# google-research/sparf

Hardware: AMD Instinct MI355X
Metric: training rays/sec (64c+128f samples, 8x256 MLP) (higher is better)
Workload: dtype bf16x3; 1 GPU; BASELINE configs[1]: DTU-shaped scene, fixed GT poses, photometric loss; 4 views 300x400, 4096 rays x (64 coarse + 128 fine) per GPU and step, fwd+bwd+clip+Adam, both 8x256 MLPs; samples=64+128, precision_mode=bf16x3, launch=eager, optimizer=clip_grad_norm(0.1) + Adam, sparf_amd.optim.FusedAdam

## Files before the change

sparf_amd/build.py:

```python
import os
import subprocess
import sys

HERE = os.path.dirname(os.path.abspath(__file__))
CSRC = os.path.join(HERE, "csrc")
OUT = os.path.join(HERE, "libsparf_hip.so")
FUSED_UNITS = ["mlp_fwd_fp32_train.hip", "mlp_fwd_fp32_infer.hip", "rays_fwd_fp32.hip", "rays_bwd_fp32.hip", "mlp_fwd_x3_train.hip", "rays_fwd_x3.hip", "mlp_fwd_x3_train_q8.hip", "mlp_fwd_x3_infer.hip", "mlp_bwd.hip", "mlp_bwd_fp32.hip", "mlp_bwd_x3.hip", "mlp_bwd_x3w4.hip", "mlp_bwd_q8.hip", "rays_bwd_x3.hip", "rays_bwd_x3w4.hip", "rays_bwd.hip", "rays_fwd_bf16.hip",
               "mlp_fwd_bf16_train.hip", "mlp_fwd_bf16_train_q8.hip", "mlp_fwd_bf16_infer.hip"]
RAYS_UNITS = ["rays_fwd_fp32.hip", "rays_bwd_fp32.hip", "rays_fwd_x3.hip", "rays_bwd_x3.hip", "rays_bwd_x3w4.hip", "rays_bwd.hip", "rays_fwd_bf16.hip"]
MLP_DISPATCH = "mlp_launch.hip"
SOURCES = FUSED_UNITS + ["wgrad.hip", "api.hip", MLP_DISPATCH, "ray_ops.hip", "pose.hip", "pose_eval.hip", "reproj.hip", "dcons.hip", "photo.hip", "matches.hip", "colmap.hip", "depth_err.hip", "pick.hip", "metrics.hip", "pack.hip", "optim.hip", "calib.hip", "tables.cpp"]
HEADERS = ["layout.h", "streams.h", "mlp_dev.h", "mlp_fwd_impl.h", "mlp_bwd_impl.h", "kernels.h", "pass_plan.h", "ordered.h", "reproj.h", "dcons.h", "photo.h", "matches.h", "colmap.h", "depth_err.h", "pick.h", "metrics.h", "pose_eval.h", "rigid.h", os.path.join("..", "..", "include", "sparf_hip.h")]
FLAGS = ["--offload-arch=gfx950", "-O3", "-std=c++17", "-fPIC", "-ffp-contract=on", "-fconstexpr-steps=200000000"]


def source_hash():
    import hashlib
    h = hashlib.sha1()
    for f in sorted(SOURCES) + sorted(HEADERS):
        h.update(open(os.path.join(CSRC, f), "rb").read())
    return h.hexdigest()[:16]


def _deps(path, seen=None):
    import re
    seen = set() if seen is None else seen
    if path in seen or not os.path.exists(path):
        return seen
    seen.add(path)
    for inc in re.findall(r'^\s*#\s*include\s+"([^"]+)"', open(path, errors="replace").read(), flags=re.M):
        _deps(os.path.normpath(os.path.join(os.path.dirname(path), inc)), seen)
    return seen


def _newer(target, deps):
    if not os.path.exists(target):
        return True
    t = os.path.getmtime(target)
    return any(os.path.getmtime(d) > t for d in deps)


def build(force=False, verbose=True, out=None, extra_flags=(), tag="", only=None):
    hipcc = os.environ.get("HIPCC", "/opt/rocm/bin/hipcc")
    bdir = os.path.join(CSRC, "build" + tag)
    out = out or OUT
    os.makedirs(bdir, exist_ok=True)
    hdrs = [os.path.join(CSRC, h) for h in HEADERS]
    procs, objs = [], []
    for src in SOURCES:
        sp = os.path.join(CSRC, src)
        if only is not None and src not in only:
            objs.append(os.path.join(CSRC, "build", os.path.splitext(src)[0] + ".o"))
            continue
        obj = os.path.join(bdir, os.path.splitext(src)[0] + ".o")
        objs.append(obj)
        if force or _newer(obj, sorted(_deps(sp))):
            cmd = [hipcc] + FLAGS + list(extra_flags) + (["-x", "hip"] if src.endswith(".cpp") else []) + ["-c", sp, "-o", obj]
            if verbose:
                print("[sparf_amd.build]", " ".join(cmd), flush=True)
            procs.append((src, subprocess.Popen(cmd, stdout=subprocess.PIPE, stderr=subprocess.STDOUT, text=True)))
    failed = []
    for src, p in procs:
        log, _ = p.communicate()
        if p.returncode != 0:
            failed.append((src, log))
# ... 14 lines not shown
```

sparf_amd/csrc/optim.hip:

```cpp
#include "kernels.h"
#include "layout.h"

namespace sparf {

enum { OPT_BLOCK = 256, OPT_PARTS = 256 };

__global__ void __launch_bounds__(OPT_BLOCK) grad_sqnorm_kernel(const float* __restrict__ g, int n, float* __restrict__ parts, int* __restrict__ step_dev) {
    if (step_dev && blockIdx.x == 0 && threadIdx.x == 0) *step_dev += 1;
    if (!parts) return;
    float s = 0.f;
    for (int i = blockIdx.x * OPT_BLOCK + threadIdx.x; i < n; i += OPT_PARTS * OPT_BLOCK) s += g[i] * g[i];
    __shared__ float red[OPT_BLOCK];
    red[threadIdx.x] = s;
    __syncthreads();
    for (int k = OPT_BLOCK / 2; k > 0; k >>= 1) {
        if ((int)threadIdx.x < k) red[threadIdx.x] += red[threadIdx.x + k];
        __syncthreads();
    }
    if (threadIdx.x == 0) parts[blockIdx.x] = red[0];
}

struct OptPtrs { float* p[2 * N_LAYERS]; };

struct AdamArgs {
    OptPtrs p;
    const float* grad;
    float* exp_avg;
    float* exp_avg_sq;
    const float* parts;
    float* norm_out;
    float lr, beta1, beta2, eps, bias1, bias2_sqrt, max_norm;
    const int* step_dev;
};

__global__ void __launch_bounds__(OPT_BLOCK) adam_kernel(AdamArgs a) {
    __shared__ int off[2 * N_LAYERS + 1];
    __shared__ float* ptr[2 * N_LAYERS];
    __shared__ float clip, sh_bias1, sh_bias2_sqrt;
    if (threadIdx.x == 1) {
        float b1 = a.bias1, b2s = a.bias2_sqrt;
        if (a.step_dev) {
            const double st = (double)*a.step_dev;
            b1 = (float)(1.0 - pow((double)a.beta1, st));
            b2s = (float)sqrt(1.0 - pow((double)a.beta2, st));
        }
        sh_bias1 = b1; sh_bias2_sqrt = b2s;
    }
    if (threadIdx.x < 2 * N_LAYERS + 1) {
        const int k = threadIdx.x;
        off[k] = k == 2 * N_LAYERS ? (int)N_PARAMS : (int)((k & 1) ? param_b_off(k >> 1) : param_w_off(k >> 1));
    }
#pragma unroll
    for (int k = 0; k < 2 * N_LAYERS; ++k)
        if ((int)threadIdx.x == k + 32) ptr[k] = a.p.p[k];
    if (threadIdx.x == 0) {
        float c = 1.0f;
        if (a.parts) {
            float s = 0.f;
            for (int i = 0; i < OPT_PARTS; ++i) s += a.parts[i];
            const float norm = sqrtf(s);
            c = fminf(a.max_norm / (norm + 1e-6f), 1.0f);
            if (a.norm_out && blockIdx.x == 0) *a.norm_out = norm;
        }
        clip = c;
    }
    __syncthreads();
    const int i = blockIdx.x * OPT_BLOCK + threadIdx.x;
    if (i >= N_PARAMS) return;
    int k = 0;
#pragma unroll
    for (int step = 16; step > 0; step >>= 1)
        if (k + step <= 2 * N_LAYERS && off[k + step] <= i) k += step;
    float* w = ptr[k] + (i - off[k]);
    const float g = a.grad[i] * clip;
    const float m = a.exp_avg[i] + (1.0f - a.beta1) * (g - a.exp_avg[i]);
    const float v = a.beta2 * a.exp_avg_sq[i] + (1.0f - a.beta2) * g * g;
    a.exp_avg[i] = m;
    a.exp_avg_sq[i] = v;
    const float denom = sqrtf(v) / sh_bias2_sqrt + a.eps;
    *w = *w - (a.lr / sh_bias1) * (m / denom);
}

int launch_adam(const float* const* params, const float* grad, float* exp_avg, float* exp_avg_sq, float* workspace, float* norm_out,
                float lr, float beta1, float beta2, float eps, int step, int* step_dev, float max_norm, hipStream_t s) {
    AdamArgs a;
    for (int i = 0; i < 2 * N_LAYERS; ++i) a.p.p[i] = const_cast<float*>(params[i]);
    a.grad = grad; a.exp_avg = exp_avg; a.exp_avg_sq = exp_avg_sq;
    a.parts = nullptr; a.norm_out = norm_out;
    a.lr = lr; a.beta1 = beta1; a.beta2 = beta2; a.eps = eps; a.max_norm = max_norm;
    a.step_dev = step_dev;
    a.bias1 = (float)(1.0 - pow((double)beta1, (double)(step > 0 ? step : 1)));
    a.bias2_sqrt = (float)sqrt(1.0 - pow((double)beta2, (double)(step > 0 ? step : 1)));
    if (max_norm > 0.0f || step_dev) {
        hipLaunchKernelGGL(grad_sqnorm_kernel, dim3(max_norm > 0.0f ? OPT_PARTS : 1), dim3(OPT_BLOCK), 0, s, grad, (int)N_PARAMS,
                           max_norm > 0.0f ? workspace : (float*)nullptr, step_dev);
        if (max_norm > 0.0f) a.parts = workspace;
    }
    hipLaunchKernelGGL(adam_kernel, dim3((N_PARAMS + OPT_BLOCK - 1) / OPT_BLOCK), dim3(OPT_BLOCK), 0, s, a);
    return hipGetLastError() == hipSuccess ? 0 : 2;
}


enum { PHOTO_BLOCK = 1024, PHOTO_PARTS = 256, PHOTO_SINGLE_MAX = 65536 };

__global__ void __launch_bounds__(PHOTO_BLOCK) photometric_loss_kernel(const float* __restrict__ pred, const float* __restrict__ pred_fine,
                                                                       const float* __restrict__ target, int64_t n, int kind, float delta,
                                                                       float* __restrict__ out, float* __restrict__ d_pred,
                                                                       float* __restrict__ d_pred_fine, int final_scale) {
    const float inv = kind == 0 ? (float)(1.0 / ((double)n + 1e-6)) : (float)(2.0 / (double)n);
    float s = 0.f;
    for (int64_t i = (int64_t)blockIdx.x * PHOTO_BLOCK + threadIdx.x; i < n; i += (int64_t)gridDim.x * PHOTO_BLOCK) {
        const float t = target[i];
#pragma unroll
        for (int f = 0; f < 2; ++f) {
            const float* p = f ? pred_fine : pred;
            float* d = f ? d_pred_fine : d_pred;
            if (!p) continue;
            const float e = p[i] - t;
            float l, g;
            if (kind == 0) { l = e * e; g = 2.0f * e; }
            else if (fabsf(e) <= delta) { l = 0.5f * e * e; g = e; }
            else { l = delta * (fabsf(e) - 0.5f * delta); g = e > 0.f ? delta : -delta; }
            s += l;
            if (d) d[i] = g * inv;
        }
    }
    __shared__ float red[PHOTO_BLOCK];
    red[threadIdx.x] = s;
    __syncthreads();
    for (int k = PHOTO_BLOCK / 2; k > 0; k >>= 1) {
        if ((int)threadIdx.x < k) red[threadIdx.x] += red[threadIdx.x + k];
        __syncthreads();
    }
    if (threadIdx.x == 0) out[blockIdx.x] = final_scale ? red[0] * inv : red[0];
}

__global__ void __launch_bounds__(PHOTO_PARTS) photometric_final_kernel(const float* __restrict__ parts, int nparts, int64_t n, int kind,
                                                                        float* __restrict__ loss) {
    __shared__ float red[PHOTO_PARTS];
    red[threadIdx.x] = (int)threadIdx.x < nparts ? parts[threadIdx.x] : 0.f;
    __syncthreads();
    for (int k = PHOTO_PARTS / 2; k > 0; k >>= 1) {
        if ((int)threadIdx.x < k) red[threadIdx.x] += red[threadIdx.x + k];
        __syncthreads();
    }
    if (threadIdx.x == 0) *loss = red[0] * (kind == 0 ? (float)(1.0 / ((double)n + 1e-6)) : (float)(2.0 / (double)n));
}

int photometric_workspace_floats() { return PHOTO_PARTS; }

int launch_photometric_loss(const float* pred, const float* pred_fine, const float* target, int64_t n, int kind, float delta,
// ... 17 lines not shown
```

sparf_amd/csrc/ray_ops.hip:

```cpp
#include "kernels.h"
#include "mlp_dev.h"

namespace sparf {

static SP_DEV double wave_incl_scan(double v, int lane) {
#pragma unroll
    for (int d = 1; d < 64; d <<= 1) {
        double o = __shfl_up(v, d);
        if (lane >= d) v += o;
    }
    return v;
}
static SP_DEV double wave_rev_incl_scan(double v, int lane) {
#pragma unroll
    for (int d = 1; d < 64; d <<= 1) {
        double o = __shfl_down(v, d);
        if (lane + d < 64) v += o;
    }
    return v;
}
static SP_DEV double wave_sum(double v) {
#pragma unroll
    for (int d = 32; d >= 1; d >>= 1) v += __shfl_xor(v, d);
    return v;
}
static SP_DEV float wave_sumf(float v) {
#pragma unroll
    for (int d = 32; d >= 1; d >>= 1) v += __shfl_xor(v, d);
    return v;
}
static SP_DEV float softplus_f(float x) { return x > 20.0f ? x : log1pf(expf(x)); }
static SP_DEV float sigmoid_f(float x) { return 1.0f / (1.0f + expf(-x)); }

template <int PREC>
__global__ void ray_setup_kernel(const float* __restrict__ dir, int nrays, const float* __restrict__ c2f_view,
                                 typename Policy<PREC>::stage_t* __restrict__ venc, float* __restrict__ raylen) {
    typedef typename Policy<PREC>::stage_t act_t;
    constexpr int CH = Policy<PREC>::CH;
    int ray = blockIdx.x * blockDim.x + threadIdx.x;
    if (ray >= nrays) return;
    float x = dir[ray * 3], y = dir[ray * 3 + 1], z = dir[ray * 3 + 2];
    float len = sqrtf(__fadd_rn(__fadd_rn(__fmul_rn(x, x), __fmul_rn(y, y)), __fmul_rn(z, z)));
    raylen[ray] = len;
    float inv = fmaxf(len, 1e-12f);
    float d[3] = {x / inv, y / inv, z / inv};
    float feat[V_DIM];
    feat[0] = d[0]; feat[1] = d[1]; feat[2] = d[2];
    for (int c = 0; c < 3; ++c)
        for (int k = 0; k < LVIEW; ++k) {
            float s, co;
            sincosf(__fmul_rn(d[c], pe_freq(k)), &s, &co);
            feat[3 + c * 8 + k] = __fmul_rn(s, c2f_view[k]);
            feat[3 + c * 8 + 4 + k] = __fmul_rn(co, c2f_view[k]);
        }
    act_t* o = venc + (int64_t)ray * 32;
    for (int h = 0; h < 2; ++h)
        for (int q = 0; q < 16; ++q) {
            int f = view_feat(q, h);
            o[pos_of(q, h, CH)] = (act_t)(f < 0 ? 0.0f : feat[f]);
        }
}

__global__ void sample_coarse_kernel(const float* __restrict__ jitter, float u_const, const float* __restrict__ dmax_ray,
                                     const float* __restrict__ range_dev, float dmin, float scale, int inverse, int64_t rows,
                                     int nsamp, float* __restrict__ t) {
    int64_t i = (int64_t)blockIdx.x * blockDim.x + threadIdx.x;
    if (i >= rows) return;
    if (range_dev) {
        dmin = range_dev[0];
        if (!dmax_ray) scale = __fsub_rn(range_dev[1], dmin);
    }
    int s = (int)(i % nsamp);
    float u = jitter ? jitter[i] : u_const;
    float sc = dmax_ray ? __fsub_rn(dmax_ray[i / nsamp], dmin) : scale;
    float v = __fadd_rn(__fmul_rn(__fdiv_rn(__fadd_rn(u, (float)s), (float)nsamp), sc), dmin);
    if (inverse) v = __fdiv_rn(1.0f, __fadd_rn(v, 1e-8f));
    t[i] = v;
}

struct SegPick {
    int ray0; float noise_scale; const float *g_rgb, *g_depth, *g_opacity, *g_weights;
    const float *g_depth_var, *g_rgb_var, *g_all_cum, *g_density, *g_rgb_samples;
};
static SP_DEV SegPick pick_segment(const SegTable& st, int ray, const SegPick& pass_level) {
    SegPick p = pass_level;
    if (st.n > 0) {
#pragma unroll
        for (int s = 0; s < MAX_SEGMENTS; ++s)
            if (s < st.n && ray >= st.ray0[s])
                p = SegPick{st.ray0[s], st.noise_scale[s], st.g_rgb[s], st.g_depth[s], st.g_opacity[s], st.g_weights[s],
                            st.g_depth_var[s], st.g_rgb_var[s], st.g_all_cum[s], st.g_density[s], st.g_rgb_samples[s]};
    }
    return p;
}

__global__ void __launch_bounds__(64) composite_fwd_kernel(CompositeFwdArgs a) {
    const int ray = blockIdx.x, lane = threadIdx.x;
    const int N = a.nsamp;
    const int64_t base = (int64_t)ray * N;
    const float ell = a.raylen[ray];
    const float noise_scale = pick_segment(a.seg, ray, SegPick{0, a.noise_scale, nullptr, nullptr, nullptr, nullptr, nullptr, nullptr, nullptr, nullptr, nullptr}).noise_scale;
    double carry = 0.0;
    float s_w = 0.f, s_d = 0.f, s_r = 0.f, s_g = 0.f, s_b = 0.f;
    float T_nm2 = 1.0f;
    for (int j0 = 0; j0 < N; j0 += 64) {
        const int i = j0 + lane;
        const bool ok = i < N;
        float sd = 0.f, tt = 0.f, dens = 0.f;
        if (ok) {
            tt = a.t[base + i];
            float tn = i + 1 < N ? a.t[base + i + 1] : 0.f;
            float delta = i + 1 < N ? __fsub_rn(tn, tt) : 1e10f;
            float raw = a.sigma_raw[base + i];
            if (a.noise && noise_scale != 0.0f) raw = __fadd_rn(raw, __fmul_rn(a.noise[base + i], noise_scale));
            dens = a.direct ? raw : softplus_f(raw);
            sd = __fmul_rn(dens, __fmul_rn(delta, ell));
        }
        double incl = wave_incl_scan((double)sd, lane);
        double excl = carry + incl - (double)sd;
        carry += __shfl(incl, 63);
        if (ok) {
            float T = expf(-(float)excl);
            float alpha = 1.0f - expf(-sd);
            float w = T * alpha;
            a.weights[base + i] = w;
            if (a.density) a.density[base + i] = dens;
            if (i == N - 2) T_nm2 = T;
            const float* c = a.rgb_samples + (base + i) * 3;
            s_w += w; s_d += w * tt; s_r += w * c[0]; s_g += w * c[1]; s_b += w * c[2];
        }
    }
    const float opacity = wave_sumf(s_w), depth = wave_sumf(s_d);
    const float r = wave_sumf(s_r), g = wave_sumf(s_g), b = wave_sumf(s_b);
    float Tn = (N >= 2 && ((N - 2) % 64) == lane) ? T_nm2 : 0.f;
    Tn = wave_sumf(Tn);
    float v_d = 0.f, v_c = 0.f;
    for (int j0 = 0; j0 < N; j0 += 64) {
        const int i = j0 + lane;
        if (i < N) {
            float w = a.weights[base + i], tt = a.t[base + i];
            const float* c = a.rgb_samples + (base + i) * 3;
            float dd = tt - depth;
            v_d += w * dd * dd;
            v_c += w * ((c[0] - r) + (c[1] - g) + (c[2] - b));
        }
    }
    v_d = wave_sumf(v_d); v_c = wave_sumf(v_c);
    if (lane == 0) {
        float add = a.white_bg ? 1.0f - opacity : 0.0f;
        a.rgb[ray * 3 + 0] = r + add; a.rgb[ray * 3 + 1] = g + add; a.rgb[ray * 3 + 2] = b + add;
        a.depth[ray] = depth; a.opacity[ray] = opacity; a.depth_var[ray] = v_d; a.rgb_var[ray] = v_c;
        a.all_cumulated[ray] = Tn;
    }
}

__global__ void __launch_bounds__(64) composite_bwd_kernel(CompositeBwdArgs a) {
    const int ray = a.ray_base + blockIdx.x, lane = threadIdx.x;
    const int N = a.nsamp;
    const int64_t base = (int64_t)ray * N;
    const float ell = a.raylen[ray];
    const SegPick sg = pick_segment(a.seg, ray, SegPick{0, a.noise_scale, a.g_rgb, a.g_depth, a.g_opacity, a.g_weights,
                                                      a.g_depth_var, a.g_rgb_var, a.g_all_cum, a.g_density, a.g_rgb_samples});
    const int lray = ray - sg.ray0;
    const float noise_scale = sg.noise_scale;
    const float* gw = sg.g_weights ? sg.g_weights + (int64_t)lray * N : nullptr;
    const float* gdn = sg.g_density ? sg.g_density + (int64_t)lray * N : nullptr;
    const float* grs = sg.g_rgb_samples ? sg.g_rgb_samples + (int64_t)lray * N * 3 : nullptr;
    float gC[3] = {0.f, 0.f, 0.f}, gD = 0.f, gO = 0.f;
    if (sg.g_rgb) { gC[0] = sg.g_rgb[lray * 3]; gC[1] = sg.g_rgb[lray * 3 + 1]; gC[2] = sg.g_rgb[lray * 3 + 2]; }
    if (sg.g_depth) gD = sg.g_depth[lray];
    if (sg.g_opacity) gO = sg.g_opacity[lray];
    if (a.white_bg) gO -= gC[0] + gC[1] + gC[2];
    const float gV = sg.g_depth_var ? sg.g_depth_var[lray] : 0.f, gU = sg.g_rgb_var ? sg.g_rgb_var[lray] : 0.f;
    const float gA = sg.g_all_cum ? sg.g_all_cum[lray] : 0.f;
    float Dr = 0.f, Or = 0.f, SC = 0.f;
    if (sg.g_depth_var || sg.g_rgb_var) {
        for (int i = lane; i < N; i += 64) {
            const float w = a.weights[base + i];
            const float* c = a.rgb_samples + (base + i) * 3;
            Dr += w * a.t[base + i]; Or += w; SC += w * (c[0] + c[1] + c[2]);
        }
        Dr = wave_sumf(Dr); Or = wave_sumf(Or); SC = wave_sumf(SC);
    }
    double carry_sd = 0.0;
    float A_part = 0.f;
    for (int j0 = 0; j0 < N; j0 += 64) {
        const int i = j0 + lane;
        float sd = 0.f;
        if (i < N) {
            const float tt = a.t[base + i];
            const float delta = i + 1 < N ? __fsub_rn(a.t[base + i + 1], tt) : 1e10f;
            float raw = a.sigma_raw[base + i];
            if (a.noise && noise_scale != 0.0f) raw = __fadd_rn(raw, __fmul_rn(a.noise[base + i], noise_scale));
            sd = __fmul_rn(a.direct ? raw : softplus_f(raw), __fmul_rn(delta, ell));
        }
        double incl_sd = carry_sd + wave_incl_scan((double)sd, lane);
        carry_sd = __shfl(incl_sd, 63);
        if (i < N) {
            const float Tn = expf(-(float)incl_sd);
            a.d_sigma_raw[base + i] = Tn;
            if (i == N - 3) A_part = Tn;
        }
    }
    const float A = sg.g_all_cum ? (N >= 3 ? wave_sumf(A_part) : N == 2 ? 1.0f : 0.0f) : 0.0f;
    double carry = 0.0;
    float dlen = 0.f;
    for (int j0 = ((N - 1) / 64) * 64; j0 >= 0; j0 -= 64) {
        const int i = j0 + lane;
        const bool ok = i < N;
        float w = 0.f, q = 0.f, tt = 0.f, dens = 0.f, delta = 0.f, raw = 0.f, Tn1 = 0.f;
        const float* c = a.rgb_samples + (base + (ok ? i : 0)) * 3;
        if (ok) {
            tt = a.t[base + i];
            w = a.weights[base + i];
            q = gC[0] * c[0] + gC[1] * c[1] + gC[2] * c[2] + gD * tt + gO + (gw ? gw[i] : 0.f);
            if (sg.g_depth_var) q += gV * ((tt - Dr) * (tt - Dr) - 2.0f * tt * Dr * (1.0f - Or));
            if (sg.g_rgb_var) q += gU * ((c[0] + c[1] + c[2]) * (1.0f - Or) - SC);
            float tn = i + 1 < N ? a.t[base + i + 1] : 0.f;
            delta = i + 1 < N ? __fsub_rn(tn, tt) : 1e10f;
            raw = a.sigma_raw[base + i];
            if (a.noise && noise_scale != 0.0f) raw = __fadd_rn(raw, __fmul_rn(a.noise[base + i], noise_scale));
            dens = a.direct ? raw : softplus_f(raw);
            Tn1 = a.d_sigma_raw[base + i];
        }
        const double wq = (double)w * (double)q;
        const double rincl = wave_rev_incl_scan(wq, lane);
        const double rnext = __shfl_down(rincl, 1);
        const double suffix_d = carry + (lane < 63 ? rnext : 0.0);
        carry += __shfl(rincl, 0);
        if (ok) {
            float suffix = (float)suffix_d;
            float ds = Tn1 * q - suffix;
            if (i < N - 2) ds -= gA * A;
            float dist = delta * ell;
            float dsig = ds * dist + (gdn ? gdn[i] : 0.f);
            float draw = a.direct ? dsig : dsig * (raw > 20.0f ? 1.0f : sigmoid_f(raw));
            a.d_sigma_raw[base + i] = draw;
            dlen += ds * dens * delta;
            float* dz = a.d_z + (base + i) * 3;
            const float wu = w * gU * (1.0f - Or);
#pragma unroll
            for (int ch = 0; ch < 3; ++ch) {
                const float dc = w * gC[ch] + wu + (grs ? grs[i * 3 + ch] : 0.f);
                dz[ch] = a.direct ? dc : dc * c[ch] * (1.0f - c[ch]);
            }
        }
    }
    dlen = wave_sumf(dlen);
    if (lane == 0 && a.d_len) a.d_len[ray] = dlen;
}

static SP_DEV float linspace_at(float start, float end, int steps, int i) {
    float step = (end - start) / (float)(steps - 1);
    return i < steps / 2 ? __fadd_rn(start, __fmul_rn(step, (float)i)) : __fsub_rn(end, __fmul_rn(step, (float)(steps - i - 1)));
}

__global__ void __launch_bounds__(64) sample_fine_kernel(SampleFineArgs a) {
    extern __shared__ float sm[];
    const int ray = blockIdx.x, lane = threadIdx.x;
    const int Nc = a.n_coarse, Nf = a.n_fine, Nt = Nc + Nf;
    float* cdf = sm;
    float* srt = sm + (Nc + 1);
    int P = 1;
    while (P < Nt) P <<= 1;
    const float* w = a.weights + (int64_t)ray * Nc;
    const float dmin = a.range_dev ? a.range_dev[0] : a.dmin, dmax = a.range_dev ? a.range_dev[1] : a.dmax;
    double tot = 0.0;
    for (int i = lane; i < Nc; i += 64) tot += (double)w[i];
    const float denom = __fadd_rn((float)wave_sum(tot), 1e-6f);
    double carry = 0.0;
    if (lane == 0) cdf[0] = 0.f;
    for (int j0 = 0; j0 < Nc; j0 += 64) {
        const int i = j0 + lane;
        float pdf = i < Nc ? __fdiv_rn(w[i], denom) : 0.f;
        double incl = carry + wave_incl_scan((double)pdf, lane);
        carry = __shfl(incl, 63);
        if (i < Nc) cdf[i + 1] = (float)incl;
    }
    __syncthreads();
    const float* tc = a.t_coarse + (int64_t)ray * Nc;
    for (int i = lane; i < Nc; i += 64) srt[i] = tc[i];
    for (int j = lane; j < Nf; j += 64) {
        const float u = a.u_mid ? a.u_mid[j] : a.u_host[j];
        int lo = 0, hi = Nc + 1;
        while (lo < hi) {
            int mid = (lo + hi) >> 1;
            if (cdf[mid] <= u) lo = mid + 1; else hi = mid;
        }
        const int il = lo - 1 < 0 ? 0 : lo - 1, ih = lo > Nc ? Nc : lo;
        const float dl = linspace_at(dmin, dmax, Nc + 1, il), dh = linspace_at(dmin, dmax, Nc + 1, ih);
        const float cl = cdf[il], chh = cdf[ih];
        const float frac = __fdiv_rn(__fsub_rn(u, cl), __fadd_rn(__fsub_rn(chh, cl), 1e-8f));
        const float tf = __fadd_rn(dl, __fmul_rn(frac, __fsub_rn(dh, dl)));
        srt[Nc + j] = tf;
        if (a.t_fine) a.t_fine[(int64_t)ray * Nf + j] = tf;
    }
    for (int i = Nt + lane; i < P; i += 64) srt[i] = __builtin_inff();
    __syncthreads();
    for (int k = 2; k <= P; k <<= 1)
        for (int j = k >> 1; j > 0; j >>= 1) {
            for (int i = lane; i < P; i += 64) {
                int p = i ^ j;
                if (p > i) {
                    float x = srt[i], y = srt[p];
                    bool up = (i & k) == 0;
                    if ((x > y) == up) { srt[i] = y; srt[p] = x; }
                }
            }
            __syncthreads();
        }
    float* out = a.t_out + (int64_t)ray * Nt;
    for (int i = lane; i < Nt; i += 64) out[i] = srt[i];
}

__global__ void __launch_bounds__(64) ray_reduce_kernel(RayReduceArgs a) {
    const int ray = a.ray_base + blockIdx.x, lane = threadIdx.x;
    const int N = a.nsamp;
    const int64_t base = (int64_t)ray * N;
    float sc[3] = {0, 0, 0}, sr[3] = {0, 0, 0};
    for (int i = lane; i < N; i += 64) {
        const float* dp = a.dp + (base + i) * 3;
        float tt = a.t[base + i];
#pragma unroll
        for (int c = 0; c < 3; ++c) { sc[c] += dp[c]; sr[c] += tt * dp[c]; }
    }
#pragma unroll
    for (int c = 0; c < 3; ++c) { sc[c] = wave_sumf(sc[c]); sr[c] = wave_sumf(sr[c]); }
    float dvf = 0.f;
    if (a.dv) {
        const int hh = lane >> 5, col = lane & 31;
        float s0 = 0.f, s1 = 0.f, s2 = 0.f, s3 = 0.f;
        int i = hh;
        for (; i + 6 < N; i += 8) {
            s0 += a.dv[(base + i) * 32 + col];
            s1 += a.dv[(base + i + 2) * 32 + col];
            s2 += a.dv[(base + i + 4) * 32 + col];
            s3 += a.dv[(base + i + 6) * 32 + col];
        }
        for (; i < N; i += 2) s0 += a.dv[(base + i) * 32 + col];
        dvf = (s0 + s1) + (s2 + s3);
        dvf += __shfl_down(dvf, 32);
    }
    float x = a.dir[ray * 3], y = a.dir[ray * 3 + 1], z = a.dir[ray * 3 + 2];
    float len = a.raylen[ray];
    float inv = fmaxf(len, 1e-12f);
    float d[3] = {x / inv, y / inv, z / inv};
    float gd[3] = {0, 0, 0};
    if (a.dv) {
        float contrib = 0.f;
        int coord = -1;
        const int feat = lane < 32 ? view_feat(q_of_pos(lane, 4), h_of_pos(lane, 4)) : -1;
        if (feat >= 0 && feat < 3) { coord = feat; contrib = dvf; }
        else if (feat >= 3) {
            int f = feat - 3; coord = f / 8;
            int k = f % 4; bool is_cos = (f % 8) >= 4;
            float s, co;
            sincosf(__fmul_rn(d[coord], pe_freq(k)), &s, &co);
            float m = a.c2f_view[k] * pe_freq(k);
            contrib = dvf * m * (is_cos ? -s : co);
        }
#pragma unroll
        for (int c = 0; c < 3; ++c) gd[c] = wave_sumf(coord == c ? contrib : 0.f);
    }
    if (lane == 0) {
// ... 61 lines not shown
}

int launch_far_transplant(int main_prec, bool masks, const void* far_area, void* main_area, int64_t frows, int far_count, int nsamp, hipStream_t s) {
    if (frows <= 0) return 0;
    if (main_prec == PREC_FP32) return 1;
    const int64_t ntiles = (frows + 31) / 32;
    hipLaunchKernelGGL(far_transplant_kernel, dim3((unsigned)ntiles), dim3(256), 0, s, (const char*)far_area, (char*)main_area, frows, far_count, nsamp,
                       save_tile_bytes(masks ? (int)AREA_MASKS : main_prec), save_mask_tile_off(masks ? (int)AREA_MASKS : main_prec, 0), masks ? 1 : 0);
    return hipGetLastError() == hipSuccess ? 0 : 2;
}

__global__ void ray_len_kernel(const float* __restrict__ dir, int nrays, float* __restrict__ raylen) {
    int ray = blockIdx.x * blockDim.x + threadIdx.x;
    if (ray >= nrays) return;
    float x = dir[ray * 3], y = dir[ray * 3 + 1], z = dir[ray * 3 + 2];
    raylen[ray] = sqrtf(__fadd_rn(__fadd_rn(__fmul_rn(x, x), __fmul_rn(y, y)), __fmul_rn(z, z)));
}
__global__ void len_to_dir_kernel(const float* __restrict__ dir, const float* __restrict__ raylen, const float* __restrict__ d_len, int nrays,
                                  float* __restrict__ d_dir) {
    int ray = blockIdx.x * blockDim.x + threadIdx.x;
    if (ray >= nrays) return;
    const float inv = fmaxf(raylen[ray], 1e-12f), g = d_len[ray];
#pragma unroll
    for (int c = 0; c < 3; ++c) d_dir[ray * 3 + c] = g * dir[ray * 3 + c] / inv;
}
int launch_len_to_dir(const float* dir, const float* raylen, const float* d_len, int nrays, float* d_dir, hipStream_t s) {
    if (nrays <= 0) return 0;
    hipLaunchKernelGGL(len_to_dir_kernel, dim3((nrays + 255) / 256), dim3(256), 0, s, dir, raylen, d_len, nrays, d_dir);
    return hipGetLastError() == hipSuccess ? 0 : 2;
}

int launch_ray_setup(int prec, const float* dir, int nrays, const float* c2f_view, void* venc, float* raylen, hipStream_t s) {
    if (nrays <= 0) return 0;
    dim3 g((nrays + 255) / 256), b(256);
    if (prec < 0) {
        hipLaunchKernelGGL(ray_len_kernel, g, b, 0, s, dir, nrays, raylen);
        return hipGetLastError() == hipSuccess ? 0 : 2;
    }
    if (prec == PREC_BF16) hipLaunchKernelGGL(ray_setup_kernel<PREC_BF16>, g, b, 0, s, dir, nrays, c2f_view, (__bf16*)venc, raylen);
    else if (prec == PREC_FP32) hipLaunchKernelGGL(ray_setup_kernel<PREC_FP32>, g, b, 0, s, dir, nrays, c2f_view, (float*)venc, raylen);
    else if (prec == PREC_X3) hipLaunchKernelGGL(ray_setup_kernel<PREC_X3>, g, b, 0, s, dir, nrays, c2f_view, (float*)venc, raylen);
    else return 1;
    return hipGetLastError() == hipSuccess ? 0 : 2;
}
int launch_sample_coarse(const float* jitter, float u_const, const float* dmax_ray, const float* range_dev, float dmin, float scale,
                         int inverse, int64_t rows, int nsamp, float* t, hipStream_t s) {
    if (rows <= 0) return 0;
    hipLaunchKernelGGL(sample_coarse_kernel, dim3((unsigned)((rows + 255) / 256)), dim3(256), 0, s, jitter, u_const, dmax_ray, range_dev,
                       dmin, scale, inverse, rows, nsamp, t);
    return hipGetLastError() == hipSuccess ? 0 : 2;
}
int launch_composite_fwd(const CompositeFwdArgs& a, hipStream_t s) {
    if (a.nrays <= 0) return 0;
    hipLaunchKernelGGL(composite_fwd_kernel, dim3(a.nrays), dim3(64), 0, s, a);
    return hipGetLastError() == hipSuccess ? 0 : 2;
}
int launch_composite_bwd(const CompositeBwdArgs& a, hipStream_t s) {
    if (a.nrays <= 0) return 0;
    hipLaunchKernelGGL(composite_bwd_kernel, dim3(a.nrays), dim3(64), 0, s, a);
    return hipGetLastError() == hipSuccess ? 0 : 2;
}
int launch_sample_fine(const SampleFineArgs& a, hipStream_t s) {
    if (a.nrays <= 0) return 0;
    int P = 1;
    while (P < a.n_coarse + a.n_fine) P <<= 1;
    size_t smem = (size_t)(a.n_coarse + 1 + P) * sizeof(float);
    if (smem > 64 * 1024) return 3;
    hipLaunchKernelGGL(sample_fine_kernel, dim3(a.nrays), dim3(64), smem, s, a);
    return hipGetLastError() == hipSuccess ? 0 : 2;
}
int launch_ray_reduce(const RayReduceArgs& a, hipStream_t s) {
    if (a.nrays <= 0) return 0;
    hipLaunchKernelGGL(ray_reduce_kernel, dim3(a.nrays), dim3(64), 0, s, a);
    return hipGetLastError() == hipSuccess ? 0 : 2;
}


struct RayGeom { float ki[9], ri[9], ti[3]; };

static SP_DEV RayGeom ray_geom(const float* pose, const float* intr, int b) {
    RayGeom g;
    const float* K = intr + b * 9;
    const double a = K[0], bb = K[1], c = K[2], d = K[3], e = K[4], f = K[5], gg = K[6], h = K[7], i = K[8];
    const double A = e * i - f * h, B = -(d * i - f * gg), C = d * h - e * gg;
    const double det = a * A + bb * B + c * C, inv = 1.0 / det;
    g.ki[0] = (float)(A * inv); g.ki[1] = (float)(-(bb * i - c * h) * inv); g.ki[2] = (float)((bb * f - c * e) * inv);
    g.ki[3] = (float)(B * inv); g.ki[4] = (float)((a * i - c * gg) * inv);  g.ki[5] = (float)(-(a * f - c * d) * inv);
    g.ki[6] = (float)(C * inv); g.ki[7] = (float)(-(a * h - bb * gg) * inv); g.ki[8] = (float)((a * e - bb * d) * inv);
    const float* P = pose + b * 12;
#pragma unroll
    for (int r = 0; r < 3; ++r)
#pragma unroll
        for (int q = 0; q < 3; ++q) g.ri[r * 3 + q] = P[q * 4 + r];
#pragma unroll
    for (int r = 0; r < 3; ++r) g.ti[r] = -(g.ri[r * 3] * P[3] + g.ri[r * 3 + 1] * P[7] + g.ri[r * 3 + 2] * P[11]);
    return g;
}

static SP_DEV void ray_pixel(const RayGenArgs& a, int b, int r, float& x, float& y) {
    const int64_t src = (a.per_image ? (int64_t)b * a.nrays : 0) + r;
    if (a.pixels) {
        x = a.pixels[src * 2];
        y = a.pixels[src * 2 + 1];
    } else {
        const int64_t idx = a.ray_idx[src];
        x = (float)(idx % a.width) + 0.5f;
        y = (float)(idx / a.width) + 0.5f;
    }
}

__global__ void ray_gen_fwd_kernel(RayGenArgs a) {
    const int b = blockIdx.y;
// ... 72 lines not shown
```

Baseline: 626,400 rays/s.

## Vectorize Adam, register-resident multi-ray compositing, merge-based fine sample sort

Adam now handles four elements per thread with 16-byte vector loads and stores, and the first wave reads the gradient-norm partials in parallel instead of one thread summing them serially. Forward and backward compositing are templated on the number of 64-sample chunks, keep per-sample data in registers, and pack four rays per workgroup; sample counts above 256 fall back to the old loop kernel. Fine sampling replaces the full bitonic sort of coarse plus fine samples with a check that both runs are already sorted, followed by a binary-search merge-rank scatter, and keeps the bitonic sort as a fallback. These changes target launch granularity, repeated global reads and sort work, at the cost of more register pressure and extra code paths.

```diff
diff --git a/sparf_amd/build.py b/sparf_amd/build.py
--- a/sparf_amd/build.py
+++ b/sparf_amd/build.py
@@ -10,7 +10,7 @@
 RAYS_UNITS = ["rays_fwd_fp32.hip", "rays_bwd_fp32.hip", "rays_fwd_x3.hip", "rays_bwd_x3.hip", "rays_bwd_x3w4.hip", "rays_bwd.hip", "rays_fwd_bf16.hip"]
 MLP_DISPATCH = "mlp_launch.hip"
 SOURCES = FUSED_UNITS + ["wgrad.hip", "api.hip", MLP_DISPATCH, "ray_ops.hip", "pose.hip", "pose_eval.hip", "reproj.hip", "dcons.hip", "photo.hip", "matches.hip", "colmap.hip", "depth_err.hip", "pick.hip", "metrics.hip", "pack.hip", "optim.hip", "calib.hip", "tables.cpp"]
-HEADERS = ["layout.h", "streams.h", "mlp_dev.h", "mlp_fwd_impl.h", "mlp_bwd_impl.h", "kernels.h", "pass_plan.h", "ordered.h", "reproj.h", "dcons.h", "photo.h", "matches.h", "colmap.h", "depth_err.h", "pick.h", "metrics.h", "pose_eval.h", "rigid.h", os.path.join("..", "..", "include", "sparf_hip.h")]
+HEADERS = ["layout.h", "streams.h", "mlp_dev.h", "mlp_fwd_impl.h", "mlp_bwd_impl.h", "kernels.h", "pass_plan.h", "ordered.h", "merge_rank.h", "reproj.h", "dcons.h", "photo.h", "matches.h", "colmap.h", "depth_err.h", "pick.h", "metrics.h", "pose_eval.h", "rigid.h", os.path.join("..", "..", "include", "sparf_hip.h")]
 FLAGS = ["--offload-arch=gfx950", "-O3", "-std=c++17", "-fPIC", "-ffp-contract=on", "-fconstexpr-steps=200000000"]
 
 
diff --git a/sparf_amd/csrc/merge_rank.h b/sparf_amd/csrc/merge_rank.h
--- /dev/null
+++ b/sparf_amd/csrc/merge_rank.h
@@ -0,0 +1,18 @@
+#pragma once
+#include "layout.h"
+
+namespace sparf {
+
+SP_HD bool merge_run_ok(float v, bool last, float next) { return v == v && v != 0.0f && (last || v <= next); }
+
+SP_HD int merge_rank(const float* run, int n, float v, bool strict) {
+    int lo = 0, hi = n;
+    while (lo < hi) {
+        const int mid = (lo + hi) >> 1;
+        const float x = run[mid];
+        if (strict ? x < v : x <= v) lo = mid + 1; else hi = mid;
+    }
+    return lo;
+}
+
+}
diff --git a/sparf_amd/csrc/optim.hip b/sparf_amd/csrc/optim.hip
--- a/sparf_amd/csrc/optim.hip
+++ b/sparf_amd/csrc/optim.hip
@@ -3,7 +3,9 @@
 
 namespace sparf {
 
-enum { OPT_BLOCK = 256, OPT_PARTS = 256 };
+enum { OPT_BLOCK = 256, OPT_PARTS = 256, ADAM_VEC = 4 };
+static_assert(N_PARAMS % ADAM_VEC == 0, "adam_kernel reads whole vectors of the flat buffers");
+static_assert(OPT_PARTS % 64 == 0, "adam_kernel's first wave holds the partials, OPT_PARTS / 64 a lane");
 
 __global__ void __launch_bounds__(OPT_BLOCK) grad_sqnorm_kernel(const float* __restrict__ g, int n, float* __restrict__ parts, int* __restrict__ step_dev) {
     if (step_dev && blockIdx.x == 0 && threadIdx.x == 0) *step_dev += 1;
@@ -33,11 +35,54 @@
     const int* step_dev;
 };
 
+typedef float f32x4 __attribute__((ext_vector_type(4)));
+
+static __device__ __forceinline__ float adam_element(const AdamArgs& a, float clip, float bias1, float bias2_sqrt, float grad, float w, float& exp_avg, float& exp_avg_sq) {
+    const float g = grad * clip;
+    const float m = exp_avg + (1.0f - a.beta1) * (g - exp_avg);
+    const float v = a.beta2 * exp_avg_sq + (1.0f - a.beta2) * g * g;
+    exp_avg = m;
+    exp_avg_sq = v;
+    const float denom = sqrtf(v) / bias2_sqrt + a.eps;
+    return w - (a.lr / bias1) * (m / denom);
+}
+
+static __device__ __forceinline__ bool aligned16(const void* p) { return ((uintptr_t)p & 15) == 0; }
+
 __global__ void __launch_bounds__(OPT_BLOCK) adam_kernel(AdamArgs a) {
     __shared__ int off[2 * N_LAYERS + 1];
     __shared__ float* ptr[2 * N_LAYERS];
     __shared__ float clip, sh_bias1, sh_bias2_sqrt;
-    if (threadIdx.x == 1) {
+    const int tid = threadIdx.x;
+    const int i0 = (blockIdx.x * OPT_BLOCK + tid) * ADAM_VEC;
+    const bool live = i0 < N_PARAMS;
+    const bool flat16 = aligned16(a.grad) && aligned16(a.exp_avg) && aligned16(a.exp_avg_sq);
+    f32x4 g = {0.f, 0.f, 0.f, 0.f}, m = g, v = g;
+    if (live) {
+        if (flat16) {
+            g = *(const f32x4*)(a.grad + i0); m = *(const f32x4*)(a.exp_avg + i0); v = *(const f32x4*)(a.exp_avg_sq + i0);
+        } else {
+#pragma unroll
+            for (int e = 0; e < ADAM_VEC; ++e) { g[e] = a.grad[i0 + e]; m[e] = a.exp_avg[i0 + e]; v[e] = a.exp_avg_sq[i0 + e]; }
+        }
+    }
+    if (tid < 64) {
+        float c = 1.0f;
+        if (a.parts) {
+            float pv[OPT_PARTS / 64];
+#pragma unroll
+            for (int j = 0; j < OPT_PARTS / 64; ++j) pv[j] = a.parts[j * 64 + tid];
+            float s = 0.f;
+#pragma unroll
+            for (int j = 0; j < OPT_PARTS / 64; ++j)
+#pragma unroll
+                for (int l = 0; l < 64; ++l) s += __int_as_float(__builtin_amdgcn_readlane(__float_as_int(pv[j]), l));
+            const float norm = sqrtf(s);
+            c = fminf(a.max_norm / (norm + 1e-6f), 1.0f);
+            if (tid == 0 && a.norm_out && blockIdx.x == 0) *a.norm_out = norm;
+        }
+        if (tid == 0) clip = c;
+    } else if (tid == 64) {
         float b1 = a.bias1, b2s = a.bias2_sqrt;
         if (a.step_dev) {
             const double st = (double)*a.step_dev;
@@ -45,40 +90,55 @@
             b2s = (float)sqrt(1.0 - pow((double)a.beta2, st));
         }
         sh_bias1 = b1; sh_bias2_sqrt = b2s;
-    }
-    if (threadIdx.x < 2 * N_LAYERS + 1) {
-        const int k = threadIdx.x;
+    } else if (tid >= 128 && tid < 128 + 2 * N_LAYERS + 1) {
+        const int k = tid - 128;
         off[k] = k == 2 * N_LAYERS ? (int)N_PARAMS : (int)((k & 1) ? param_b_off(k >> 1) : param_w_off(k >> 1));
     }
 #pragma unroll
     for (int k = 0; k < 2 * N_LAYERS; ++k)
-        if ((int)threadIdx.x == k + 32) ptr[k] = a.p.p[k];
-    if (threadIdx.x == 0) {
-        float c = 1.0f;
-        if (a.parts) {
-            float s = 0.f;
-            for (int i = 0; i < OPT_PARTS; ++i) s += a.parts[i];
-            const float norm = sqrtf(s);
-            c = fminf(a.max_norm / (norm + 1e-6f), 1.0f);
-            if (a.norm_out && blockIdx.x == 0) *a.norm_out = norm;
-        }
-        clip = c;
-    }
-    __syncthreads();
-    const int i = blockIdx.x * OPT_BLOCK + threadIdx.x;
-    if (i >= N_PARAMS) return;
+        if (tid == k + 192) ptr[k] = a.p.p[k];
+    __syncthreads();
+    if (!live) return;
+    const float cl = clip, bias1 = sh_bias1, bias2_sqrt = sh_bias2_sqrt;
     int k = 0;
 #pragma unroll
     for (int step = 16; step > 0; step >>= 1)
-        if (k + step <= 2 * N_LAYERS && off[k + step] <= i) k += step;
-    float* w = ptr[k] + (i - off[k]);
-    const float g = a.grad[i] * clip;
-    const float m = a.exp_avg[i] + (1.0f - a.beta1) * (g - a.exp_avg[i]);
-    const float v = a.beta2 * a.exp_avg_sq[i] + (1.0f - a.beta2) * g * g;
-    a.exp_avg[i] = m;
-    a.exp_avg_sq[i] = v;
-    const float denom = sqrtf(v) / sh_bias2_sqrt + a.eps;
-    *w = *w - (a.lr / sh_bias1) * (m / denom);
+        if (k + step <= 2 * N_LAYERS && off[k + step] <= i0) k += step;
+    if (i0 + ADAM_VEC <= off[k + 1]) {
+        float* w = ptr[k] + (i0 - off[k]);
+        const bool w16 = aligned16(w);
+        f32x4 wv;
+        if (w16) wv = *(const f32x4*)w;
+        else {
+#pragma unroll
+            for (int e = 0; e < ADAM_VEC; ++e) wv[e] = w[e];
+        }
+#pragma unroll
+        for (int e = 0; e < ADAM_VEC; ++e) {
+            float me = m[e], ve = v[e];
+            wv[e] = adam_element(a, cl, bias1, bias2_sqrt, g[e], wv[e], me, ve);
+            m[e] = me; v[e] = ve;
+        }
+        if (w16) *(f32x4*)w = wv;
+        else {
+#pragma unroll
+            for (int e = 0; e < ADAM_VEC; ++e) w[e] = wv[e];
+        }
+    } else {
+#pragma unroll
+        for (int e = 0; e < ADAM_VEC; ++e) {
+            while (off[k + 1] <= i0 + e) ++k;
+            float* w = ptr[k] + (i0 + e - off[k]);
+            float me = m[e], ve = v[e];
+            *w = adam_element(a, cl, bias1, bias2_sqrt, g[e], *w, me, ve);
+            m[e] = me; v[e] = ve;
+        }
+    }
+    if (flat16) { *(f32x4*)(a.exp_avg + i0) = m; *(f32x4*)(a.exp_avg_sq + i0) = v; }
+    else {
+#pragma unroll
+        for (int e = 0; e < ADAM_VEC; ++e) { a.exp_avg[i0 + e] = m[e]; a.exp_avg_sq[i0 + e] = v[e]; }
+    }
 }
 
 int launch_adam(const float* const* params, const float* grad, float* exp_avg, float* exp_avg_sq, float* workspace, float* norm_out,
@@ -96,7 +156,7 @@
                            max_norm > 0.0f ? workspace : (float*)nullptr, step_dev);
         if (max_norm > 0.0f) a.parts = workspace;
     }
-    hipLaunchKernelGGL(adam_kernel, dim3((N_PARAMS + OPT_BLOCK - 1) / OPT_BLOCK), dim3(OPT_BLOCK), 0, s, a);
+    hipLaunchKernelGGL(adam_kernel, dim3((N_PARAMS + OPT_BLOCK * ADAM_VEC - 1) / (OPT_BLOCK * ADAM_VEC)), dim3(OPT_BLOCK), 0, s, a);
     return hipGetLastError() == hipSuccess ? 0 : 2;
 }
 
diff --git a/sparf_amd/csrc/ray_ops.hip b/sparf_amd/csrc/ray_ops.hip
--- a/sparf_amd/csrc/ray_ops.hip
+++ b/sparf_amd/csrc/ray_ops.hip
@@ -1,5 +1,6 @@
 #include "kernels.h"
 #include "mlp_dev.h"
+#include "merge_rank.h"
 
 namespace sparf {
 
@@ -94,7 +95,91 @@
     return p;
 }
 
-__global__ void __launch_bounds__(64) composite_fwd_kernel(CompositeFwdArgs a) {
+enum { COMPOSITE_REG_CHUNKS = 4, COMPOSITE_RAYS_PER_WG = 4 };
+
+template <int C>
+__global__ void __launch_bounds__(64 * COMPOSITE_RAYS_PER_WG) composite_fwd_kernel(CompositeFwdArgs a) {
+    const int lane = threadIdx.x & 63;
+    const int ray = blockIdx.x * COMPOSITE_RAYS_PER_WG + __builtin_amdgcn_readfirstlane(threadIdx.x >> 6);
+    if (ray >= a.nrays) return;
+    const int N = a.nsamp;
+    const int64_t base = (int64_t)ray * N;
+    const float ell = a.raylen[ray];
+    const float noise_scale = pick_segment(a.seg, ray, SegPick{0, a.noise_scale, nullptr, nullptr, nullptr, nullptr, nullptr, nullptr, nullptr, nullptr, nullptr}).noise_scale;
+    const bool noisy = a.noise && noise_scale != 0.0f;
+    float tt[C], tn[C], raw[C], nz[C], col[C][3];
+#pragma unroll
+    for (int k = 0; k < C; ++k) {
+        const int i = k * 64 + lane, ic = i < N ? i : N - 1;
+        tt[k] = a.t[base + ic];
+        tn[k] = a.t[base + (ic + 1 < N ? ic + 1 : ic)];
+        raw[k] = a.sigma_raw[base + ic];
+        const float* c = a.rgb_samples + (base + ic) * 3;
+        col[k][0] = c[0]; col[k][1] = c[1]; col[k][2] = c[2];
+    }
+#pragma unroll
+    for (int k = 0; k < C; ++k) {
+        const int i = k * 64 + lane;
+        nz[k] = noisy ? a.noise[base + (i < N ? i : N - 1)] : 0.f;
+    }
+    if (noisy)
+#pragma unroll
+        for (int k = 0; k < C; ++k) raw[k] = __fadd_rn(raw[k], __fmul_rn(nz[k], noise_scale));
+    double carry = 0.0;
+    float s_w = 0.f, s_d = 0.f, s_r = 0.f, s_g = 0.f, s_b = 0.f;
+    float T_nm2 = 1.0f;
+    float wv[C];
+#pragma unroll
+    for (int k = 0; k < C; ++k) {
+        const int i = k * 64 + lane;
+        const bool ok = i < N;
+        float sd = 0.f, dens = 0.f;
+        if (ok) {
+            float delta = i + 1 < N ? __fsub_rn(tn[k], tt[k]) : 1e10f;
+            dens = a.direct ? raw[k] : softplus_f(raw[k]);
+            sd = __fmul_rn(dens, __fmul_rn(delta, ell));
+        }
+        double incl = wave_incl_scan((double)sd, lane);
+        double excl = carry + incl - (double)sd;
+        carry += __shfl(incl, 63);
+        wv[k] = 0.f;
+        if (ok) {
+            float T = expf(-(float)excl);
+            float alpha = 1.0f - expf(-sd);
+            float w = T * alpha;
+            a.weights[base + i] = w;
+            if (a.density) a.density[base + i] = dens;
+            if (i == N - 2) T_nm2 = T;
+            const float* c = col[k];
+            s_w += w; s_d += w * tt[k]; s_r += w * c[0]; s_g += w * c[1]; s_b += w * c[2];
+            wv[k] = w;
+        }
+    }
+    const float opacity = wave_sumf(s_w), depth = wave_sumf(s_d);
+    const float r = wave_sumf(s_r), g = wave_sumf(s_g), b = wave_sumf(s_b);
+    float Tn = (N >= 2 && ((N - 2) % 64) == lane) ? T_nm2 : 0.f;
+    Tn = wave_sumf(Tn);
+    float v_d = 0.f, v_c = 0.f;
+#pragma unroll
+    for (int k = 0; k < C; ++k) {
+        if (k * 64 + lane < N) {
+            float w = wv[k];
+            const float* c = col[k];
+            float dd = tt[k] - depth;
+            v_d += w * dd * dd;
+            v_c += w * ((c[0] - r) + (c[1] - g) + (c[2] - b));
+        }
+    }
+    v_d = wave_sumf(v_d); v_c = wave_sumf(v_c);
+    if (lane == 0) {
+        float add = a.white_bg ? 1.0f - opacity : 0.0f;
+        a.rgb[ray * 3 + 0] = r + add; a.rgb[ray * 3 + 1] = g + add; a.rgb[ray * 3 + 2] = b + add;
+        a.depth[ray] = depth; a.opacity[ray] = opacity; a.depth_var[ray] = v_d; a.rgb_var[ray] = v_c;
+        a.all_cumulated[ray] = Tn;
+    }
+}
+
+__global__ void __launch_bounds__(64) composite_fwd_loop_kernel(CompositeFwdArgs a) {
     const int ray = blockIdx.x, lane = threadIdx.x;
     const int N = a.nsamp;
     const int64_t base = (int64_t)ray * N;
@@ -154,7 +239,128 @@
     }
 }
 
-__global__ void __launch_bounds__(64) composite_bwd_kernel(CompositeBwdArgs a) {
+template <int C>
+__global__ void __launch_bounds__(64 * COMPOSITE_RAYS_PER_WG) composite_bwd_kernel(CompositeBwdArgs a) {
+    const int lane = threadIdx.x & 63;
+    const int lr = blockIdx.x * COMPOSITE_RAYS_PER_WG + __builtin_amdgcn_readfirstlane(threadIdx.x >> 6);
+    if (lr >= a.nrays) return;
+    const int ray = a.ray_base + lr;
+    const int N = a.nsamp;
+    const int64_t base = (int64_t)ray * N;
+    const float ell = a.raylen[ray];
+    const SegPick sg = pick_segment(a.seg, ray, SegPick{0, a.noise_scale, a.g_rgb, a.g_depth, a.g_opacity, a.g_weights,
+                                                      a.g_depth_var, a.g_rgb_var, a.g_all_cum, a.g_density, a.g_rgb_samples});
+    const int lray = ray - sg.ray0;
+    const float noise_scale = sg.noise_scale;
+    const bool noisy = a.noise && noise_scale != 0.0f;
+    const float* gw = sg.g_weights ? sg.g_weights + (int64_t)lray * N : nullptr;
+    const float* gdn = sg.g_density ? sg.g_density + (int64_t)lray * N : nullptr;
+    const float* grs = sg.g_rgb_samples ? sg.g_rgb_samples + (int64_t)lray * N * 3 : nullptr;
+    float tt[C], tn[C], raw[C], nz[C], col[C][3], wv[C], gwv[C], gdv[C], grv[C][3];
+#pragma unroll
+    for (int k = 0; k < C; ++k) {
+        const int i = k * 64 + lane, ic = i < N ? i : N - 1;
+        tt[k] = a.t[base + ic];
+        tn[k] = a.t[base + (ic + 1 < N ? ic + 1 : ic)];
+        raw[k] = a.sigma_raw[base + ic];
+        const float* c = a.rgb_samples + (base + ic) * 3;
+        col[k][0] = c[0]; col[k][1] = c[1]; col[k][2] = c[2];
+        wv[k] = a.weights[base + ic];
+    }
+#pragma unroll
+    for (int k = 0; k < C; ++k) {
+        const int i = k * 64 + lane, ic = i < N ? i : N - 1;
+        nz[k] = noisy ? a.noise[base + ic] : 0.f;
+        gwv[k] = gw ? gw[ic] : 0.f;
+        gdv[k] = gdn ? gdn[ic] : 0.f;
+#pragma unroll
+        for (int ch = 0; ch < 3; ++ch) grv[k][ch] = grs ? grs[ic * 3 + ch] : 0.f;
+    }
+    if (noisy)
+#pragma unroll
+        for (int k = 0; k < C; ++k) raw[k] = __fadd_rn(raw[k], __fmul_rn(nz[k], noise_scale));
+    float gC[3] = {0.f, 0.f, 0.f}, gD = 0.f, gO = 0.f;
+    if (sg.g_rgb) { gC[0] = sg.g_rgb[lray * 3]; gC[1] = sg.g_rgb[lray * 3 + 1]; gC[2] = sg.g_rgb[lray * 3 + 2]; }
+    if (sg.g_depth) gD = sg.g_depth[lray];
+    if (sg.g_opacity) gO = sg.g_opacity[lray];
+    if (a.white_bg) gO -= gC[0] + gC[1] + gC[2];
+    const float gV = sg.g_depth_var ? sg.g_depth_var[lray] : 0.f, gU = sg.g_rgb_var ? sg.g_rgb_var[lray] : 0.f;
+    const float gA = sg.g_all_cum ? sg.g_all_cum[lray] : 0.f;
+    float Dr = 0.f, Or = 0.f, SC = 0.f;
+    if (sg.g_depth_var || sg.g_rgb_var) {
+#pragma unroll
+        for (int k = 0; k < C; ++k)
+            if (k * 64 + lane < N) {
+                const float w = wv[k];
+                const float* c = col[k];
+                Dr += w * tt[k]; Or += w; SC += w * (c[0] + c[1] + c[2]);
+            }
+        Dr = wave_sumf(Dr); Or = wave_sumf(Or); SC = wave_sumf(SC);
+    }
+    double carry_sd = 0.0;
+    float A_part = 0.f;
+    float Tn1[C], dens[C], delta[C];
+#pragma unroll
+    for (int k = 0; k < C; ++k) {
+        const int i = k * 64 + lane;
+        float sd = 0.f;
+        dens[k] = 0.f; delta[k] = 0.f; Tn1[k] = 0.f;
+        if (i < N) {
+            delta[k] = i + 1 < N ? __fsub_rn(tn[k], tt[k]) : 1e10f;
+            dens[k] = a.direct ? raw[k] : softplus_f(raw[k]);
+            sd = __fmul_rn(dens[k], __fmul_rn(delta[k], ell));
+        }
+        double incl_sd = carry_sd + wave_incl_scan((double)sd, lane);
+        carry_sd = __shfl(incl_sd, 63);
+        if (i < N) {
+            Tn1[k] = expf(-(float)incl_sd);
+            if (i == N - 3) A_part = Tn1[k];
+        }
+    }
+    const float A = sg.g_all_cum ? (N >= 3 ? wave_sumf(A_part) : N == 2 ? 1.0f : 0.0f) : 0.0f;
+    double carry = 0.0;
+    float dlen = 0.f;
+#pragma unroll
+    for (int k = C - 1; k >= 0; --k) {
+        const int i = k * 64 + lane;
+        const bool ok = i < N;
+        float w = 0.f, q = 0.f;
+        const float* c = col[k];
+        if (ok) {
+            const float tt_ = tt[k];
+            w = wv[k];
+            q = gC[0] * c[0] + gC[1] * c[1] + gC[2] * c[2] + gD * tt_ + gO + gwv[k];
+            if (sg.g_depth_var) q += gV * ((tt_ - Dr) * (tt_ - Dr) - 2.0f * tt_ * Dr * (1.0f - Or));
+            if (sg.g_rgb_var) q += gU * ((c[0] + c[1] + c[2]) * (1.0f - Or) - SC);
+        }
+        const double wq = (double)w * (double)q;
+        const double rincl = wave_rev_incl_scan(wq, lane);
+        const double rnext = __shfl_down(rincl, 1);
+        const double suffix_d = carry + (lane < 63 ? rnext : 0.0);
+        carry += __shfl(rincl, 0);
+        if (ok) {
+            float suffix = (float)suffix_d;
+            float ds = Tn1[k] * q - suffix;
+            if (i < N - 2) ds -= gA * A;
+            float dist = delta[k] * ell;
+            float dsig = ds * dist + gdv[k];
+            float draw = a.direct ? dsig : dsig * (raw[k] > 20.0f ? 1.0f : sigmoid_f(raw[k]));
+            a.d_sigma_raw[base + i] = draw;
+            dlen += ds * dens[k] * delta[k];
+            float* dz = a.d_z + (base + i) * 3;
+            const float wu = w * gU * (1.0f - Or);
+#pragma unroll
+            for (int ch = 0; ch < 3; ++ch) {
+                const float dc = w * gC[ch] + wu + grv[k][ch];
+                dz[ch] = a.direct ? dc : dc * c[ch] * (1.0f - c[ch]);
+            }
+        }
+    }
+    dlen = wave_sumf(dlen);
+    if (lane == 0 && a.d_len) a.d_len[ray] = dlen;
+}
+
+__global__ void __launch_bounds__(64) composite_bwd_loop_kernel(CompositeBwdArgs a) {
     const int ray = a.ray_base + blockIdx.x, lane = threadIdx.x;
     const int N = a.nsamp;
     const int64_t base = (int64_t)ray * N;
@@ -255,6 +461,19 @@
     return i < steps / 2 ? __fadd_rn(start, __fmul_rn(step, (float)i)) : __fsub_rn(end, __fmul_rn(step, (float)(steps - i - 1)));
 }
 
+static SP_DEV void wave_bitonic_lds(float* s, int P, int lane) {
+    for (int k = 2; k <= P; k <<= 1)
+        for (int j = k >> 1; j > 0; j >>= 1) {
+            for (int q = lane; q < (P >> 1); q += 64) {
+                const int i = ((q & ~(j - 1)) << 1) | (q & (j - 1)), p = i | j;
+                const float x = s[i], y = s[p];
+                const bool up = (i & k) == 0;
+                if ((x > y) == up) { s[i] = y; s[p] = x; }
+            }
+            __syncthreads();
+        }
+}
+
 __global__ void __launch_bounds__(64) sample_fine_kernel(SampleFineArgs a) {
     extern __shared__ float sm[];
     const int ray = blockIdx.x, lane = threadIdx.x;
@@ -297,19 +516,31 @@
     }
     for (int i = Nt + lane; i < P; i += 64) srt[i] = __builtin_inff();
     __syncthreads();
-    for (int k = 2; k <= P; k <<= 1)
-        for (int j = k >> 1; j > 0; j >>= 1) {
-            for (int i = lane; i < P; i += 64) {
-                int p = i ^ j;
-                if (p > i) {
-                    float x = srt[i], y = srt[p];
-                    bool up = (i & k) == 0;
-                    if ((x > y) == up) { srt[i] = y; srt[p] = x; }
-                }
-            }
-            __syncthreads();
-        }
     float* out = a.t_out + (int64_t)ray * Nt;
+    int Pf = 1;
+    while (Pf < Nf) Pf <<= 1;
+    bool plain = true, asc_f = true;
+    for (int i = lane; i < Nt; i += 64) {
+        const float v = srt[i];
+        const bool last = i == Nc - 1 || i == Nt - 1;
+        const float next = last ? 0.f : srt[i + 1];
+        if (i < Nc) plain = plain && merge_run_ok(v, last, next);
+        else { plain = plain && merge_run_ok(v, true, 0.f); asc_f = asc_f && merge_run_ok(v, last, next); }
+    }
+    bool merge = __all(plain);
+    if (merge && !__all(asc_f)) {
+        if (Nc + Pf <= P) wave_bitonic_lds(srt + Nc, Pf, lane);
+        else merge = false;
+    }
+    if (merge) {
+        for (int i = lane; i < Nt; i += 64) {
+            const float v = srt[i];
+            const bool coarse = i < Nc;
+            out[(coarse ? i : i - Nc) + merge_rank(coarse ? srt + Nc : srt, coarse ? Nf : Nc, v, coarse)] = v;
+        }
+        return;
+    }
+    wave_bitonic_lds(srt, P, lane);
     for (int i = lane; i < Nt; i += 64) out[i] = srt[i];
 }
 
@@ -477,12 +708,27 @@
 }
 int launch_composite_fwd(const CompositeFwdArgs& a, hipStream_t s) {
     if (a.nrays <= 0) return 0;
-    hipLaunchKernelGGL(composite_fwd_kernel, dim3(a.nrays), dim3(64), 0, s, a);
+    const dim3 g((a.nrays + COMPOSITE_RAYS_PER_WG - 1) / COMPOSITE_RAYS_PER_WG), b(64 * COMPOSITE_RAYS_PER_WG);
+    switch (a.nsamp > 0 ? (a.nsamp + 63) / 64 : 0) {
+        case 1: hipLaunchKernelGGL(composite_fwd_kernel<1>, g, b, 0, s, a); break;
+        case 2: hipLaunchKernelGGL(composite_fwd_kernel<2>, g, b, 0, s, a); break;
+        case 3: hipLaunchKernelGGL(composite_fwd_kernel<3>, g, b, 0, s, a); break;
+        case 4: hipLaunchKernelGGL(composite_fwd_kernel<4>, g, b, 0, s, a); break;
+        default: hipLaunchKernelGGL(composite_fwd_loop_kernel, dim3(a.nrays), dim3(64), 0, s, a);
+    }
+    static_assert(COMPOSITE_REG_CHUNKS == 4, "one case per chunk count");
     return hipGetLastError() == hipSuccess ? 0 : 2;
 }
 int launch_composite_bwd(const CompositeBwdArgs& a, hipStream_t s) {
     if (a.nrays <= 0) return 0;
-    hipLaunchKernelGGL(composite_bwd_kernel, dim3(a.nrays), dim3(64), 0, s, a);
+    const dim3 g((a.nrays + COMPOSITE_RAYS_PER_WG - 1) / COMPOSITE_RAYS_PER_WG), b(64 * COMPOSITE_RAYS_PER_WG);
+    switch (a.nsamp > 0 ? (a.nsamp + 63) / 64 : 0) {
+        case 1: hipLaunchKernelGGL(composite_bwd_kernel<1>, g, b, 0, s, a); break;
+        case 2: hipLaunchKernelGGL(composite_bwd_kernel<2>, g, b, 0, s, a); break;
+        case 3: hipLaunchKernelGGL(composite_bwd_kernel<3>, g, b, 0, s, a); break;
+        case 4: hipLaunchKernelGGL(composite_bwd_kernel<4>, g, b, 0, s, a); break;
+        default: hipLaunchKernelGGL(composite_bwd_loop_kernel, dim3(a.nrays), dim3(64), 0, s, a);
+    }
     return hipGetLastError() == hipSuccess ? 0 : 2;
 }
 int launch_sample_fine(const SampleFineArgs& a, hipStream_t s) {
```

New measurement: 629,800 rays/s (median of 6 runs). About the same (+0.5%).
